# svg-project/Sparse-VideoGen

Hardware: AMD Instinct MI355X
Metric: attn_tflops_svg1_block_sparse (higher is better)
Workload: dtype bf16; 1 GPU; HunyuanVideo T2V hy720p SVG1 sparse layer-call: sample_mse(64 rows) + band attention with fused head placement, cfg=1 H=24 D=128 F=33 P=3600 ctx=256 prompt=64 S=119056 band=15616 density=0.2456; parallelism=single, variant=0, heads=alt

## Files before the change

include/svg_attn.h:

```cpp
#ifndef SVG_ATTN_H_
#define SVG_ATTN_H_

#include <stddef.h>
#include <stdint.h>

#ifdef __cplusplus
extern "C" {
#endif

#define SVG_DTYPE_BF16 0
#define SVG_DTYPE_F16 1
#define SVG_DTYPE_F32 2

#define SVG_OK 0
#define SVG_ERR_BAD_ARG (-1)
#define SVG_ERR_UNSUPPORTED (-2)
#define SVG_ERR_WORKSPACE (-3)
#define SVG_ERR_LAUNCH (-4)

#define SVG_ABI_VERSION 4
int svg_abi_version(void);

const char* svg_strerror(int code);
int svg_last_hip_error(void);
// ... 212 lines not shown
int svg_sample_mse_flagged(const void* q, const void* k, const void* v, const int64_t* rows, int32_t R, int32_t BH, int32_t S,
                           int32_t D, int32_t dtype, float sm_scale, const svg_profile_desc_t* prof, float* out_mse,
                           void* workspace, size_t workspace_bytes, const int32_t* skip_flag, void* stream);

size_t svg_band_attention_fp8_workspace_bytes(int32_t BH, int32_t S, int32_t D);
int svg_band_attention_fp8(const void* q, const void* k, const void* v, void* o, int32_t BH, int32_t S, int32_t D, int32_t dtype,
                           float sm_scale, const svg_band_mask_t* mask, const svg_perm_desc_t* perm, void* workspace,
                           size_t workspace_bytes, void* stream);
int svg_band_attention_fp8_stage(const void* q, const void* k, const void* v, void* o, int32_t BH, int32_t S, int32_t D, int32_t dtype,
                                 float sm_scale, const svg_band_mask_t* mask, const svg_perm_desc_t* perm, void* workspace,
                                 size_t workspace_bytes, int32_t stage, void* stream);

size_t svg_varblock_attention_fp8_workspace_bytes(int32_t Hq, int32_t Hkv, int32_t QB, int32_t KB, int32_t Sq, int32_t Skv, int32_t D);
int svg_varblock_attention_fp8(const void* q, const void* k, const void* v, void* o, int32_t Hq, int32_t Hkv, int32_t Sq, int32_t Skv,
                               int32_t D, int32_t dtype, float sm_scale, const uint8_t* block_map, const int32_t* q_sizes,
                               const int32_t* k_sizes, int32_t QB, int32_t KB, const int32_t* q_row_idx, const int32_t* kv_row_idx,
                               void* workspace, size_t workspace_bytes, void* stream);

int32_t svg_band_attention_notify_target(int32_t S, const svg_band_mask_t* mask);
int svg_band_attention_notify(const void* q, const void* k, const void* v, void* o, int32_t BH, int32_t S, int32_t D,
                              int32_t dtype, float sm_scale, const svg_band_mask_t* mask, const svg_perm_desc_t* perm,
                              int32_t* done_per_head, int32_t done_words, void* stream);
int svg_wait_counters(const int32_t* counters, int32_t n, int32_t target, void* stream);
int svg_wait_counters_deadline(const int32_t* counters, int32_t n, int32_t target, int32_t timeout_ms, int32_t* timed_out,
                               void* stream);
int32_t svg_band_attention_notify_layout(int32_t S, const svg_band_mask_t* mask, int32_t nseg, int32_t* row_bounds, int32_t* targets);
int svg_band_attention_notify_seg(const void* q, const void* k, const void* v, void* o, int32_t BH, int32_t S, int32_t D,
                                  int32_t dtype, float sm_scale, const svg_band_mask_t* mask, const svg_perm_desc_t* perm,
                                  int32_t* done, int32_t done_words, int32_t nseg, void* stream);
int svg_band_attention_prescaled_notify_seg(const void* q_scaled, const void* k, const void* v, void* o, int32_t BH, int32_t S,
                                            int32_t D, int32_t dtype, const svg_band_mask_t* mask, const svg_perm_desc_t* perm,
                                            int32_t* done, int32_t done_words, int32_t nseg, void* stream);

int svg_debug_pp_trace(uint64_t* out104);

int svg_debug_clock_probe(const int32_t* stop_flag, uint64_t* out2, int32_t max_ms, void* stream);

int svg_debug_wg_trace(uint64_t* out, int32_t n_workgroups);

#ifdef __cplusplus
}
#endif
#endif
```

sparse-videogen_amd/csrc/attention.hip:

```cpp
#include <algorithm>

#include "attn_core.h"
#include "attn_f8.h"
#include "attn_m16.h"
#include "band_policy.h"

namespace svg {

template <typename T, int D, int NW>
__global__ __launch_bounds__(NW * 64, 2) void band_attn_kernel(typename BandPolicy<T, D, NW>::Params prm) {
    extern __shared__ __attribute__((aligned(16))) char smem[];
    attn_body<T, D, NW, BandPolicy<T, D, NW>>(prm, smem, nullptr);
}

template <typename T, int D>
__global__ __launch_bounds__(512, (D == 64 ? 4 : 2)) void band_attn_pp2_kernel(typename BandPolicy<T, D, 8>::Params prm) {
    extern __shared__ __attribute__((aligned(16))) char smem[];
    attn_body_pp2<T, D, BandPolicy<T, D, 8>, false, 0, false, D == 64>(prm, smem, nullptr);
}
template <typename T>
__global__ __launch_bounds__(512, 4) void band_attn_pp2_switch64_kernel(typename BandPolicy<T, 64, 8>::Params prm,
                                                                        typename BandPolicy<T, 64, 8>::Params prm_alt,
                                                                        const int32_t* __restrict__ flag) {
    extern __shared__ __attribute__((aligned(16))) char smem[];
    if (flag[0] != 0) attn_body_pp2<T, 64, BandPolicy<T, 64, 8>, false, 0, false, true>(prm_alt, smem, nullptr);
    else attn_body_pp2<T, 64, BandPolicy<T, 64, 8>, false, 0, false, true>(prm, smem, nullptr);
}
template <typename T, int D>
__global__ __launch_bounds__(512, 2) void band_attn_pp2q_switch_kernel(typename BandPolicy<T, D, 8>::Params prm,
                                                                       typename BandPolicy<T, D, 8>::Params prm_alt,
                                                                       const int32_t* __restrict__ flag) {
    extern __shared__ __attribute__((aligned(16))) char smem[];
    if (flag[0] != 0) attn_body_pp2<T, D, BandPolicy<T, D, 8>, false, 0, true>(prm_alt, smem, nullptr);
    else attn_body_pp2<T, D, BandPolicy<T, D, 8>, false, 0, true>(prm, smem, nullptr);
}

__global__ __launch_bounds__(512, 2) void band_attn_pp2_frozen_kernel(typename BandPolicy<__bf16, 128, 8>::Params prm) {
    extern __shared__ __attribute__((aligned(16))) char smem[];
    attn_body_pp2<__bf16, 128, BandPolicy<__bf16, 128, 8>, false, 8>(prm, smem, nullptr);
}
template <typename T>
__global__ __launch_bounds__(512, 2) void band_attn_m16_kernel(typename BandPolicy<T, 128, 8>::Params prm) {
    extern __shared__ __attribute__((aligned(16))) char smem[];
    attn_body_m16<T, BandPolicy<T, 128, 8>, false, 1>(prm, smem, nullptr);
}
template <typename T>
__global__ __launch_bounds__(512, 2) void band_attn_m16q_kernel(typename BandPolicy<T, 128, 8>::Params prm) {
    extern __shared__ __attribute__((aligned(16))) char smem[];
    attn_body_m16<T, BandPolicy<T, 128, 8>, false, 1, true>(prm, smem, nullptr);
}
template <typename T, bool PRE = false>
__global__ __launch_bounds__(512, 2) void band_attn_m16_switch_kernel(typename BandPolicy<T, 128, 8>::Params prm,
                                                                      typename BandPolicy<T, 128, 8>::Params prm_alt,
                                                                      const int32_t* __restrict__ flag) {
    extern __shared__ __attribute__((aligned(16))) char smem[];
    if (flag[0] != 0) attn_body_m16<T, BandPolicy<T, 128, 8>, false, 1, PRE>(prm_alt, smem, nullptr);
    else attn_body_m16<T, BandPolicy<T, 128, 8>, false, 1, PRE>(prm, smem, nullptr);
}
template <typename T, int D>
__global__ __launch_bounds__(512, 2) void band_attn_pp2q_kernel(typename BandPolicy<T, D, 8>::Params prm) {
    extern __shared__ __attribute__((aligned(16))) char smem[];
    attn_body_pp2<T, D, BandPolicy<T, D, 8>, false, 0, true>(prm, smem, nullptr);
}
#ifdef SVG_ABLATIONS
template <typename T, int D, int ABL>
__global__ __launch_bounds__(512, 2) void band_attn_pp2_trace_kernel(typename BandPolicy<T, D, 8>::Params prm) {
    extern __shared__ __attribute__((aligned(16))) char smem[];
    attn_body_pp2<T, D, BandPolicy<T, D, 8>, true, ABL>(prm, smem, nullptr);
}
template <typename T>
__global__ __launch_bounds__(512, 2) void band_attn_m16_trace_kernel(typename BandPolicy<T, 128, 8>::Params prm) {
    extern __shared__ __attribute__((aligned(16))) char smem[];
    attn_body_m16<T, BandPolicy<T, 128, 8>, true>(prm, smem, nullptr);
}
template <typename T, int D>
__global__ __launch_bounds__(512, 2) void band_attn_pp2q_trace_kernel(typename BandPolicy<T, D, 8>::Params prm) {
    extern __shared__ __attribute__((aligned(16))) char smem[];
    attn_body_pp2<T, D, BandPolicy<T, D, 8>, true, 0, true>(prm, smem, nullptr);
}
#endif

constexpr int kVbMaxKB = 4032;
constexpr int kVbFull = 256;
// ... 593 lines not shown
static inline int band_default(int D) { return D == 128 ? kBandM16 : kBandPingPong; }

int band_waves_per_tile(int variant) {
    const int v = variant == kBandAuto ? kBandPingPong : variant;
    return v == kBandW4 ? 4 : ((v == kBandPingPong || v == kBandM16) ? 8 : -1);
}

}

using namespace svg;

__global__ __launch_bounds__(64) void wait_counters_kernel(const int32_t* __restrict__ counters, int n, int target) {
    for (int i = threadIdx.x; i < n; i += 64) {
        while (__hip_atomic_load(counters + i, __ATOMIC_ACQUIRE, __HIP_MEMORY_SCOPE_AGENT) < target) __builtin_amdgcn_s_sleep(32);
    }
}

__global__ __launch_bounds__(64) void wait_counters_deadline_kernel(const int32_t* __restrict__ counters, int n, int target,
                                                                    long long ticks, int32_t* __restrict__ timed_out) {
    const long long t0 = wall_clock64();
    for (int i = threadIdx.x; i < n; i += 64) {
        while (__hip_atomic_load(counters + i, __ATOMIC_ACQUIRE, __HIP_MEMORY_SCOPE_AGENT) < target) {
            if (wall_clock64() - t0 > ticks) {
                __hip_atomic_store(timed_out, 1, __ATOMIC_RELAXED, __HIP_MEMORY_SCOPE_SYSTEM);
                return;
            }
            __builtin_amdgcn_s_sleep(32);
        }
    }
}

static bool g_trace_is_w4 = false;

static int band_check_args(const void* q, const void* k, const void* v, const void* o, int32_t BH, int32_t S, int32_t D,
                           const svg_band_mask_t* mask, const svg_perm_desc_t* perm) {
    if (!q || !k || !v || !o || !mask || BH <= 0 || S <= 0) return SVG_ERR_BAD_ARG;
    if (const int rc = check_band_mask(S, mask, perm); rc != SVG_OK) return rc;
    if ((int64_t)BH * S * D >= (1ll << 40)) return SVG_ERR_UNSUPPORTED;
    return check_rows(S, D);
}

static int band_dispatch(const void* q, const void* k, const void* v, void* o, int32_t BH, int32_t S, int32_t D, int32_t dtype,
                         float sm_scale, const svg_band_mask_t* mask, const svg_perm_desc_t* perm, int32_t variant, BandOpts opts,
                         int32_t done_words, const svg_attn_layout_t* layout, void* stream) {
    int rc = band_check_args(q, k, v, o, BH, S, D, mask, perm);
    if (rc == SVG_OK && opts.alt_mask) rc = check_band_mask(S, opts.alt_mask, nullptr);
    if (rc != SVG_OK) return rc;
    if (opts.done && (int64_t)done_words < (int64_t)BH * (opts.done_nseg + 1)) return SVG_ERR_WORKSPACE;
    if (opts.strided && (rc = layout_from_abi(layout, BH, BH, S, S, D, q, k, v, o, opts.lay)) != SVG_OK) return rc;
    const hipStream_t st = (hipStream_t)stream;
    int trace_abl = -1;
    if ((variant & 0xFF) == 32) {
        opts.trace = true;
        opts.trace_abl = (variant >> 8) & 15;
        g_trace_is_w4 = true;
        return run_band_w4(q, k, v, o, BH, S, D, dtype, sm_scale, mask, perm, opts, st);
    }
    if (variant & 64) {
        trace_abl = (variant >> 8) & 15;
        variant = kBandPingPong;
        g_trace_is_w4 = false;
    }
    if (variant == kBandAuto) variant = band_default(D);
    if (opts.done && band_waves_per_tile(variant) < 0) return SVG_ERR_UNSUPPORTED;
    if (opts.strided && variant != kBandM16 && variant != kBandPingPong) return SVG_ERR_UNSUPPORTED;
    if (variant == kBandW4) return run_band_w4(q, k, v, o, BH, S, D, dtype, sm_scale, mask, perm, opts, st);
    if (variant != kBandLockstep4 && variant != kBandPingPong && variant != kBandFrozen && variant != kBandM16) return SVG_ERR_BAD_ARG;
    return dispatch_td(dtype, D, [&](auto t, auto d) -> int {
        using T = decltype(t);
        constexpr int DD = decltype(d)::value;
        using Pol = BandPolicy<T, DD, 8>;
        auto launch = [&](auto kern, int lds) {
            const typename Pol::Params p = make_band_params<Pol, T>(q, k, v, o, BH, S, sm_scale, mask, perm, opts);
            return launch_attn(kern, p, dim3(p.nqt * BH), 512, lds, st);
        };
        auto launch_switch = [&](auto kern, int lds) {
            const typename Pol::Params a = make_band_params<Pol, T>(q, k, v, o, BH, S, sm_scale, mask, perm, opts);
            const typename Pol::Params b = make_band_params<Pol, T>(q, k, v, o, BH, S, sm_scale, opts.alt_mask, nullptr, opts);
            if (const int r2 = configure_lds((const void*)kern, lds); r2 != SVG_OK) return r2;
            hipLaunchKernelGGL(kern, dim3(std::max(a.nqt, b.nqt) * BH), dim3(512), lds, st, a, b, opts.use_alt);
            return launch_status();
        };
        switch (variant) {
            case kBandLockstep4: {
                using Pol4 = BandPolicy<T, DD, 4>;
                const typename Pol4::Params p = make_band_params<Pol4, T>(q, k, v, o, BH, S, sm_scale, mask, perm, opts);
                return launch_attn(band_attn_kernel<T, DD, 4>, p, dim3(p.nqt * BH), 256, attn_lds_bytes<DD, 4>(), st);
            }
            case kBandPingPong:
#ifdef SVG_ABLATIONS
                if constexpr (DD == 128 && std::is_same<T, __bf16>::value) {
                    switch (trace_abl) {
#define SVG_PP_TRACE(A) case A: return launch(band_attn_pp2_trace_kernel<T, DD, A>, attn_pp2_lds_bytes<DD>());
                        SVG_PP_TRACE(0) SVG_PP_TRACE(1) SVG_PP_TRACE(2) SVG_PP_TRACE(4) SVG_PP_TRACE(5) SVG_PP_TRACE(6) SVG_PP_TRACE(7) SVG_PP_TRACE(8)
#undef SVG_PP_TRACE
                        case -1: break;
                        case 3: return launch(band_attn_pp2q_trace_kernel<T, DD>, attn_pp2_lds_bytes<DD>());
                        case 9: return launch(band_attn_m16_trace_kernel<T>, attn_m16_lds_bytes());
                        default: return SVG_ERR_UNSUPPORTED;
                    }
                }
#endif
                if (trace_abl >= 0) return SVG_ERR_UNSUPPORTED;
                if (opts.use_alt) {
                    if (opts.prescaled) return launch_switch(band_attn_pp2q_switch_kernel<T, DD>, attn_pp2_lds_bytes<DD>());
                    if constexpr (DD == 64) return launch_switch(band_attn_pp2_switch64_kernel<T>, attn_pp2_lds_bytes<64>());
                    return SVG_ERR_UNSUPPORTED;
                }
                return launch(opts.prescaled ? band_attn_pp2q_kernel<T, DD> : band_attn_pp2_kernel<T, DD>, attn_pp2_lds_bytes<DD>());
            case kBandFrozen:
                if constexpr (DD == 128 && std::is_same<T, __bf16>::value) {
                    if (opts.done || opts.prescaled) return SVG_ERR_UNSUPPORTED;
                    return launch(band_attn_pp2_frozen_kernel, attn_pp2_lds_bytes<128>());
                }
                return SVG_ERR_UNSUPPORTED;
            default:
                if constexpr (DD == 128) {
                    if (opts.use_alt)
                        return launch_switch(opts.prescaled ? band_attn_m16_switch_kernel<T, true> : band_attn_m16_switch_kernel<T>,
                                             attn_m16_lds_bytes());
                    return launch(opts.prescaled ? band_attn_m16q_kernel<T> : band_attn_m16_kernel<T>, attn_m16_lds_bytes());
                }
                return SVG_ERR_UNSUPPORTED;
        }
    });
}

extern "C" int svg_band_attention(const void* q, const void* k, const void* v, void* o, int32_t BH, int32_t S, int32_t D,
                                  int32_t dtype, float sm_scale, const svg_band_mask_t* mask,
                                  const svg_perm_desc_t* perm, int32_t variant, void* stream) {
    return band_dispatch(q, k, v, o, BH, S, D, dtype, sm_scale, mask, perm, variant, BandOpts(), 0, nullptr, stream);
}

extern "C" int svg_band_attention_strided(const void* q, const void* k, const void* v, void* o, int32_t BH, int32_t S, int32_t D,
                                          int32_t dtype, float sm_scale, const svg_band_mask_t* mask, const svg_perm_desc_t* perm,
                                          const svg_attn_layout_t* layout, void* stream) {
    BandOpts opts;
    opts.strided = true;
    return band_dispatch(q, k, v, o, BH, S, D, dtype, sm_scale, mask, perm, kBandAuto, opts, 0, layout, stream);
}

extern "C" int svg_band_attention_prescaled(const void* q_scaled, const void* k, const void* v, void* o, int32_t BH, int32_t S,
                                            int32_t D, int32_t dtype, const svg_band_mask_t* mask, const svg_perm_desc_t* perm,
                                            void* stream) {
    BandOpts opts;
    opts.prescaled = true;
    return band_dispatch(q_scaled, k, v, o, BH, S, D, dtype, 1.f, mask, perm, kBandAuto, opts, 0, nullptr, stream);
}

extern "C" int32_t svg_band_attention_notify_target(int32_t S, const svg_band_mask_t* mask) {
    if (!mask || S <= 0) return -1;
    using Pol = svg::BandPolicy<__bf16, 128, 8>;
    const auto p = svg::make_band_params<Pol, __bf16>(nullptr, nullptr, nullptr, nullptr, 1, S, 1.f, mask, nullptr);
    return p.nqt * band_waves_per_tile(kBandAuto);
// ... 63 lines not shown
}

static BandOpts switch_opts(const svg_band_mask_t* alt_mask, const int32_t* use_alt_flag) {
    BandOpts opts;
    opts.alt_mask = alt_mask, opts.use_alt = use_alt_flag;
    return opts;
}

extern "C" int svg_band_attention_switch(const void* q, const void* k, const void* v, void* o, int32_t BH, int32_t S, int32_t D,
                                         int32_t dtype, float sm_scale, const svg_band_mask_t* mask, const svg_perm_desc_t* perm,
                                         const svg_band_mask_t* alt_mask, const int32_t* use_alt_flag, void* stream) {
    if (!alt_mask || !use_alt_flag) return SVG_ERR_BAD_ARG;
    return band_dispatch(q, k, v, o, BH, S, D, dtype, sm_scale, mask, perm, kBandAuto, switch_opts(alt_mask, use_alt_flag), 0, nullptr,
                         stream);
}

extern "C" int svg_band_attention_switch_strided(const void* q, const void* k, const void* v, void* o, int32_t BH, int32_t S, int32_t D,
                                                 int32_t dtype, float sm_scale, const svg_band_mask_t* mask, const svg_perm_desc_t* perm,
                                                 const svg_band_mask_t* alt_mask, const int32_t* use_alt_flag,
                                                 const svg_attn_layout_t* layout, void* stream) {
    if (!layout || !alt_mask || !use_alt_flag) return SVG_ERR_BAD_ARG;
    BandOpts opts = switch_opts(alt_mask, use_alt_flag);
    opts.strided = true;
    return band_dispatch(q, k, v, o, BH, S, D, dtype, sm_scale, mask, perm, kBandAuto, opts, 0, layout, stream);
}

extern "C" int svg_band_attention_switch_prescaled(const void* q_scaled, const void* k, const void* v, void* o, int32_t BH, int32_t S,
                                                   int32_t D, int32_t dtype, const svg_band_mask_t* mask, const svg_perm_desc_t* perm,
                                                   const svg_band_mask_t* alt_mask, const int32_t* use_alt_flag, void* stream) {
    if (!alt_mask || !use_alt_flag) return SVG_ERR_BAD_ARG;
    BandOpts opts = switch_opts(alt_mask, use_alt_flag);
    opts.prescaled = true;
    return band_dispatch(q_scaled, k, v, o, BH, S, D, dtype, 1.f, mask, perm, kBandAuto, opts, 0, nullptr, stream);
}

extern "C" int svg_debug_wg_trace(uint64_t* out, int n_workgroups) {
#ifdef SVG_ABLATIONS
    if (!out || n_workgroups < 0 || n_workgroups > kWgTraceMax) return SVG_ERR_BAD_ARG;
    hipError_t e = hipMemcpyFromSymbol(out, HIP_SYMBOL(g_wg_trace), (size_t)n_workgroups * 6 * sizeof(uint64_t));
    if (e != hipSuccess) {
        g_last_hip_error = (int)e;
        return SVG_ERR_LAUNCH;
    }
    return SVG_OK;
#else
    (void)out, (void)n_workgroups;
    return SVG_ERR_UNSUPPORTED;
#endif
}

extern "C" int svg_debug_pp_trace(uint64_t* out104) {
#ifdef SVG_ABLATIONS
    if (!out104) return SVG_ERR_BAD_ARG;
    if (g_trace_is_w4) return w4_read_trace(out104);
    hipError_t e = hipMemcpyFromSymbol(out104, HIP_SYMBOL(g_pp_trace), 104 * sizeof(uint64_t));
    if (e != hipSuccess) {
        g_last_hip_error = (int)e;
        return SVG_ERR_LAUNCH;
    }
    return SVG_OK;
#else
    (void)out104;
    return SVG_ERR_UNSUPPORTED;
#endif
}

// ... 228 lines not shown
```

sparse-videogen_amd/csrc/attn_m16.h:

```cpp
#pragma once
#include "attn_core.h"

namespace svg {

template <typename T>
struct Mfma16;
template <>
struct Mfma16<__bf16> {
    static __device__ __forceinline__ f32x4 mfma(bf16x8 a, bf16x8 b, f32x4 c) { return __builtin_amdgcn_mfma_f32_16x16x32_bf16(a, b, c, 0, 0, 0); }
    static __device__ __forceinline__ f32x4 mfma_keep_c(bf16x8 a, bf16x8 b, const f32x4& c) {
        f32x4 d;
        asm volatile("v_mfma_f32_16x16x32_bf16 %0, %1, %2, %3" : "=&v"(d) : "v"(a), "v"(b), "v"(c));
        return d;
    }
};
template <>
struct Mfma16<_Float16> {
    static __device__ __forceinline__ f32x4 mfma(f16x8 a, f16x8 b, f32x4 c) { return __builtin_amdgcn_mfma_f32_16x16x32_f16(a, b, c, 0, 0, 0); }
    static __device__ __forceinline__ f32x4 mfma_keep_c(f16x8 a, f16x8 b, const f32x4& c) {
        f32x4 d;
        asm volatile("v_mfma_f32_16x16x32_f16 %0, %1, %2, %3" : "=&v"(d) : "v"(a), "v"(b), "v"(c));
        return d;
    }
};

constexpr int attn_m16_lds_bytes() { return attn_pp2_lds_bytes<128>(); }

__device__ __forceinline__ float quad_group_max(float x) {
    x = vmax2(x, __shfl_xor(x, 16));
    return vmax2(x, __shfl_xor(x, 32));
}
__device__ __forceinline__ float quad_group_sum(float x) {
    x += __shfl_xor(x, 16);
    return x + __shfl_xor(x, 32);
}

template <typename T, typename P, bool TRACE = false, int ONEBAR = -1, bool PRE = false>
__device__ __forceinline__ void attn_body_m16(const typename P::Params& prm, char* smem, char* policy_lds) {
    using E = Elt<T>;
    using M = Mfma16<T>;
    using V8 = typename E::v8;
    constexpr int D = 128;
    constexpr int NW = 8;
    constexpr int KS = D / 32;
    constexpr int NDB = D / 16;
    constexpr int NS = 4;
    constexpr int kImg = kBN * D * 2;
    constexpr int kStage = 2 * kImg;
    constexpr int NP = 2;
    constexpr int kCarry = 8;
    constexpr int kPF = 8;
    constexpr bool kOneBar = ONEBAR < 0 ? P::kOneBarrier : (ONEBAR != 0);
    static_assert(P::kRowBlocks == 1 && !P::kPartialOut && !P::kFixup && P::kIntervalMask, "band / variable-block policy");
    constexpr bool MSUM = std::is_same_v<T, __bf16> && !PRE;
    constexpr float kBias = MSUM ? 10.f : 0.f;

    typename P::Ctx ctx;
    if (!P::init(prm, ctx, policy_lds)) return;

    const int tid = threadIdx.x;
    const int lane = tid & 63;
    const int wave = wave_id();
    const int g4 = lane >> 4;
    const int n16 = lane & 15;
    const bool lagging = wave >= NW / 2;
    const int nT = ctx.nT;

    const T* __restrict__ qb = P::q_base(prm, ctx);
    const T* __restrict__ kb_ = P::k_base(prm, ctx);
    const T* __restrict__ vb = P::v_base(prm, ctx);
    const unsigned lds0 = (unsigned)(size_t)smem;

    const int dma_kg = wave / 2;
    const int dma_db0 = (wave % 2) * NP;
    const int krow = 16 * dma_kg + (lane >> 2);
    typename P::KvCursor cur;
    P::kv_cursor_init(prm, ctx, cur, krow);
    const unsigned vsw = (unsigned)((lane >> 4) & 1) << 1;
    const unsigned col_v = (unsigned)(dma_db0 * 64 + (((lane & 3) ^ vsw) * 16));
    const unsigned lds_piece = lds0 + (unsigned)(dma_db0 * (kBN * 64) + dma_kg * 1024);
    int nphys = 0, nnext = 0;
    auto resolve = [&](int t, auto guard_c) {
        if constexpr (decltype(guard_c)::value) nnext = (t < nT) ? P::kv_phys(prm, ctx, cur, t, krow) : 0;
        else nnext = P::kv_phys(prm, ctx, cur, t, krow);
    };
    constexpr std::true_type kGuarded{};
    auto take = [&]() { nphys = nnext; };
    const unsigned k_rsb = (unsigned)P::k_rs(prm) * 2u, v_rsb = (unsigned)P::v_rs(prm) * 2u;
    auto dma_piece = [&](int t, auto j_c) {
        constexpr int j = decltype(j_c)::value;
        const unsigned st = __builtin_amdgcn_readfirstlane(lds_piece + (unsigned)((t % NS) * kStage) + j * (kBN * 64));
        const unsigned ko = __umul24((unsigned)nphys, k_rsb) + col_v;
// ... 316 lines not shown
            }
#pragma unroll
        for (int b = 0; b < 4; ++b) asm volatile("" : "+v"(sc[b][0]), "+v"(sc[b][1]));
#pragma unroll
        for (int i = 0; i < kCarry; ++i) carry_load(0, i);
    }
    const int bar_n = lagging ? 1 : 0, bar_m = lagging ? 0 : 1;
    auto tile = [&](int t, auto has_next_c, auto guard_c) {
        tick(std::integral_constant<int, 0>{});
        if constexpr (kOneBar) pp_barrier_if(bar_n);
        else pp_barrier();
        tick(std::integral_constant<int, 1>{});
        vector_phase(t, guard_c);
        tick(std::integral_constant<int, 2>{});
        if constexpr (kOneBar) pp_barrier_if(bar_m);
        else pp_barrier();
        tick(std::integral_constant<int, 3>{});
        __builtin_amdgcn_s_setprio(1);
        matrix_phase(t, has_next_c);
        __builtin_amdgcn_s_setprio(0);
    };
    int t = 0;
    for (const int n_main = nT - dist - 1; t < n_main; ++t) tile(t, std::true_type{}, std::false_type{});
    for (; t + 1 < nT; ++t) tile(t, std::true_type{}, kGuarded);
    if (nT > 0) tile(nT - 1, std::false_type{}, kGuarded);
    pp_barrier();
    if (!kOneBar && !lagging) pp_barrier();
    if constexpr (TRACE) {
        if (blockIdx.x == kPpTraceBlock && lane == 0) {
#pragma unroll
            for (int j = 0; j < 4; ++j) g_pp_trace[wave * 8 + j] = tr_acc[j];
            if (wave == 0) g_pp_trace[64] = (unsigned long long)nT, g_pp_trace[65] = tr_last - tr_first;
        }
    }

    constexpr int kEpiStride = D * 2 + 8;
    char* erow = smem + (size_t)(wave * 32) * kEpiStride;
#pragma unroll
    for (int rb = 0; rb < 2; ++rb) {
        const float l_tot = MSUM ? acc_l[rb][0] : quad_group_sum(l_run[rb]);
        const float inv = l_tot > 0.f ? 1.f / l_tot : 0.f;
#pragma unroll
        for (int db = 0; db < NDB; ++db) {
            typename E::v4 o4;
#pragma unroll
            for (int j = 0; j < 4; ++j) o4[j] = E::from_float(acc_o[db][rb][j] * inv);
            *(typename E::v4*)(erow + (rb * 16 + n16) * kEpiStride + (16 * db + 4 * g4) * 2) = o4;
        }
    }
    __builtin_amdgcn_s_waitcnt(0xc07f);
    __builtin_amdgcn_wave_barrier();
    T* __restrict__ ob = P::o_base(prm, ctx);
    const int o_rs = P::o_rs(prm);
    constexpr int kLanesPerRow = D * 2 / 8;
    constexpr int kRowsPerPass = 64 / kLanesPerRow;
    const int sub = lane / kLanesPerRow;
    const int colb = (lane - sub * kLanesPerRow) * 8;
    int ephys[32 / kRowsPerPass];
#pragma unroll
    for (int i = 0; i < 32 / kRowsPerPass; ++i) ephys[i] = P::q_phys(prm, ctx, wave * 32 + i * kRowsPerPass + sub);
#pragma unroll
    for (int i = 0; i < 32 / kRowsPerPass; ++i) {
        const int rr = i * kRowsPerPass + sub;
        const u32x2 val = *(const u32x2*)(erow + rr * kEpiStride + colb);
        if (ephys[i] >= 0) *(u32x2*)((char*)(ob + (size_t)ephys[i] * o_rs) + colb) = val;
    }
    P::notify(prm, ctx);
}

}
```

sparse-videogen_amd/csrc/band_policy.h:

```cpp
#pragma once
#include <algorithm>

#include "attn_core.h"

namespace svg {

struct BandOpts {
    int32_t* done = nullptr;
    int done_nseg = 1;
    bool prescaled = false;
    bool trace = false;
    int trace_abl = 0;
    bool strided = false;
    AttnLayout lay{};
    const svg_band_mask_t* alt_mask = nullptr;
    const int32_t* use_alt = nullptr;
};

inline int check_band_mask(int S, const svg_band_mask_t* mask, const svg_perm_desc_t* perm) {
    if (mask->real_len < 0 || mask->real_len > S || mask->band < 0 || mask->band > S + 1) return SVG_ERR_BAD_ARG;
    if (mask->colfull_lo > mask->colfull_hi || mask->rowfull_lo > mask->rowfull_hi) return SVG_ERR_BAD_ARG;
    if (perm && perm->head_perm_flag) {
        if (perm->num_frame <= 0 || perm->frame_size <= 0 || perm->vid0 < 0 ||
            (int64_t)perm->vid0 + (int64_t)perm->num_frame * perm->frame_size > S)
// ... 47 lines not shown
    static __device__ __forceinline__ int phys_row(const Params& p, const Ctx& c, int logical) {
        if (c.perm) {
            const unsigned i = (unsigned)(logical - p.vid0);
            if (i < (unsigned)p.V) {
                const unsigned pp = i / (unsigned)p.F;
                const unsigned f = i - pp * (unsigned)p.F;
                return p.vid0 + (int)(f * (unsigned)p.P + pp);
            }
        }
        return logical;
    }

    static __device__ __forceinline__ bool init(const Params& p, Ctx& c, char*) {
        int qt;
        const int nh = p.BH * p.n_heavy;
        const int b = blockIdx.x;
        if (b >= p.nqt * p.BH) return false;
        if (b < nh) {
            c.head = b / p.n_heavy;
            qt = p.heavy_lo + (b - c.head * p.n_heavy);
        } else {
            const int b2 = b - nh;
            const int full = ((p.nqt * p.BH - nh) / (kNumXCD * 32)) * (kNumXCD * 32);
            int w2 = b2;
            if (b2 < full) {
                const int xcd = b2 % kNumXCD, s = b2 / kNumXCD;
                w2 = (s / 32) * (kNumXCD * 32) + xcd * 32 + (s % 32);
            }
            const int nl = p.nqt - p.n_heavy;
            c.head = w2 / nl;
            const int r = w2 - c.head * nl;
            qt = r < p.heavy_lo ? r : r + p.n_heavy;
        }
        const bool r1 = qt >= p.reg_t0[1], r2 = qt >= p.reg_t0[2], r3 = qt >= p.reg_t0[3];
        const int rlo = r3 ? p.reg_lo[3] : r2 ? p.reg_lo[2] : r1 ? p.reg_lo[1] : p.reg_lo[0];
        const int rhi = r3 ? p.reg_hi[3] : r2 ? p.reg_hi[2] : r1 ? p.reg_hi[1] : p.reg_hi[0];
        const int rt0 = r3 ? p.reg_t0[3] : r2 ? p.reg_t0[2] : r1 ? p.reg_t0[1] : 0;
        c.qt = qt;
        c.q0 = rlo + (qt - rt0) * BM;
        c.q_end = min(rhi, c.q0 + BM);
        c.perm = (p.head_flag != nullptr) && (p.head_flag[c.head] != 0);

        constexpr int BIG = 1 << 28;
        int alo = BIG, ahi = BIG, blo = BIG, bhi = BIG, clo = BIG, chi = BIG;
        const int real = p.real_len;
        if (c.q0 < real) {
            const int qr1 = min(c.q_end, real);
            if (c.q0 < p.rf_hi && qr1 > p.rf_lo) {
                alo = 0, ahi = (real + kBN - 1) / kBN;
            } else {
                alo = max(0, c.q0 - p.band + 1) / kBN;
                ahi = (min(real, qr1 - 1 + p.band) + kBN - 1) / kBN;
                const int ch = min(p.cf_hi, real);
                if (ch > p.cf_lo) blo = p.cf_lo / kBN, bhi = (ch + kBN - 1) / kBN;
            }
        }
        if (c.q_end > real) clo = real / kBN, chi = (p.S + kBN - 1) / kBN;
#define SVG_CSWAP(x, xh, y, yh) if (y < x) { int t_ = x; x = y; y = t_; t_ = xh; xh = yh; yh = t_; }
        SVG_CSWAP(alo, ahi, blo, bhi)
        SVG_CSWAP(blo, bhi, clo, chi)
        SVG_CSWAP(alo, ahi, blo, bhi)
#undef SVG_CSWAP
        if (blo < BIG && blo <= ahi) {
            ahi = max(ahi, bhi);
            blo = clo, bhi = chi, clo = BIG, chi = BIG;
            if (blo < BIG && blo <= ahi) ahi = max(ahi, bhi), blo = BIG, bhi = BIG;
        } else if (clo < BIG && clo <= bhi) {
            bhi = max(bhi, chi), clo = BIG, chi = BIG;
        }
        c.seg_lo[0] = alo, c.seg_n[0] = ahi - alo;
        c.seg_lo[1] = blo, c.seg_n[1] = bhi - blo;
        c.seg_lo[2] = clo, c.seg_n[2] = chi - clo;
        c.nT = c.seg_n[0] + c.seg_n[1] + c.seg_n[2];
        const int w0 = c.q0 + wave_id() * kWR, w1 = min(w0 + kWR, c.q_end);
        c.fk_lo = 1, c.fk_hi = 0;
        if (w0 < c.q_end && w1 <= real) {
            const bool full_rows = w0 >= p.rf_lo && w1 <= p.rf_hi;
            c.fk_lo = full_rows ? 0 : max(w1 - p.band, 0);
            c.fk_hi = min(full_rows ? real : w0 + p.band - kBN, min(real, p.S) - kBN);
        }
        return true;
    }

    static __device__ __forceinline__ const T* q_base(const Params& p, const Ctx& c) { return p.q + layout_head_off(p.lay.q_bs, p.lay.q_hs, p.lay.hpb_q, c.head); }
    static __device__ __forceinline__ const T* k_base(const Params& p, const Ctx& c) { return p.k + layout_head_off(p.lay.k_bs, p.lay.k_hs, p.lay.hpb_kv, c.head); }
    static __device__ __forceinline__ const T* v_base(const Params& p, const Ctx& c) { return p.v + layout_head_off(p.lay.v_bs, p.lay.v_hs, p.lay.hpb_kv, c.head); }
    static __device__ __forceinline__ T* o_base(const Params& p, const Ctx& c) { return p.o + layout_head_off(p.lay.o_bs, p.lay.o_hs, p.lay.hpb_q, c.head); }
    static __device__ __forceinline__ int q_rs(const Params& p) { return p.lay.q_rs; }
    static __device__ __forceinline__ int k_rs(const Params& p) { return p.lay.k_rs; }
    static __device__ __forceinline__ int v_rs(const Params& p) { return p.lay.v_rs; }
    static __device__ __forceinline__ int o_rs(const Params& p) { return p.lay.o_rs; }

    static __device__ __forceinline__ int q_logical(const Ctx& c, int row) { return c.q0 + row; }
    static __device__ __forceinline__ bool wave_active(const Ctx& c, int wrow0) { return c.q0 + wrow0 < c.q_end; }
    static __device__ __forceinline__ int q_phys(const Params& p, const Ctx& c, int row) {
        const int l = c.q0 + row;
        return l < c.q_end ? phys_row(p, c, l) : -1;
    }
    static __device__ __forceinline__ int tile_key0(const Ctx& c, int t) {
        const int n01 = c.seg_n[0] + c.seg_n[1];
        const int a = c.seg_lo[0] + t, b = c.seg_lo[1] + (t - c.seg_n[0]), d = c.seg_lo[2] + (t - n01);
        const int bd = t < n01 ? b : d;
        return (t < c.seg_n[0] ? a : bd) * kBN;
    }
    struct TileCur {
        int k0, left;
        int k1, left1;
        int k2, left2;
    };
    static __device__ __forceinline__ void tile_cur_shift(TileCur& tc) {
        tc.k0 = tc.k1, tc.left = tc.left1;
        tc.k1 = tc.k2, tc.left1 = tc.left2;
        tc.left2 = 0;
    }
// ... 116 lines not shown
                                                         unsigned& blen) {
        const int real = p.real_len;
        const bool rq = q < real;
        const bool rowf = (unsigned)(q - p.rf_lo) < (unsigned)(p.rf_hi - p.rf_lo);
        const int band_lo = max(q - p.band + 1, 0), band_hi = min(q + p.band, real);
        const int lo = rq ? (rowf ? 0 : band_lo) : real;
        const int hi = rq ? (rowf ? real : band_hi) : p.S;
        a0 = lo, alen = (unsigned)max(hi - lo, 0);
        const int ch = min(p.cf_hi, real);
        b0 = p.cf_lo, blen = (rq && !rowf) ? (unsigned)max(ch - p.cf_lo, 0) : 0u;
    }
    static __device__ __forceinline__ float score_fixup(const Params&, float s) { return s; }
    static __device__ __forceinline__ void notify(const Params& p, const Ctx& c) {
        if (p.done) {
            asm volatile("s_waitcnt vmcnt(0)" ::: "memory");
            __threadfence();
            if ((threadIdx.x & 63) == 0) {
                int32_t* cnt = p.done + c.head * p.done_nseg;
                if (!c.perm) {
                    atomicAdd(cnt + min(c.qt / p.done_tps, p.done_nseg - 1), 1);
                } else if (atomicAdd(p.done + p.BH * p.done_nseg + c.head, 1) == p.nqt * NW - 1) {
                    __threadfence();
                    for (int sgm = 0; sgm < p.done_nseg; ++sgm) {
                        const int t_lo = sgm * p.done_tps;
                        const int t_hi = (sgm == p.done_nseg - 1) ? p.nqt : min(p.nqt, (sgm + 1) * p.done_tps);
                        atomicAdd(cnt + sgm, (t_hi - t_lo) * NW);
                    }
                }
            }
        }
    }
};

inline int configure_lds(const void* kernel, int lds) {
    struct Entry {
        const void* kernel;
        int device, lds;
    };
    static thread_local Entry table[64];
    static thread_local int n = 0;
    int dev = 0;
    if (hipGetDevice(&dev) != hipSuccess) dev = 0;
    Entry* e = nullptr;
    for (int i = 0; i < n; ++i)
        if (table[i].kernel == kernel && table[i].device == dev) e = &table[i];
    if (e && e->lds >= lds) return SVG_OK;
    const hipError_t err = hipFuncSetAttribute(kernel, hipFuncAttributeMaxDynamicSharedMemorySize, lds);
    if (err != hipSuccess) {
        g_last_hip_error = (int)err;
        return SVG_ERR_LAUNCH;
    }
    if (e) e->lds = lds;
    else if (n < 64) table[n++] = Entry{kernel, dev, lds};
    return SVG_OK;
}

template <typename K, typename Prm>
inline int launch_attn(K kernel, const Prm& prm, dim3 grid, int threads, int lds, hipStream_t st) {
    const int rc = configure_lds((const void*)kernel, lds);
    if (rc != SVG_OK) return rc;
    hipLaunchKernelGGL(kernel, grid, dim3(threads), lds, st, prm);
    return launch_status();
}

template <typename Pol, typename T>
inline typename Pol::Params make_band_params(const void* q, const void* k, const void* v, void* o, int BH, int S, float sm_scale,
// ... 57 lines not shown
```

sparse-videogen_amd/svg/_native.py:

```python
from __future__ import annotations

import ctypes as C
import os
from pathlib import Path
from typing import NamedTuple, Optional, Sequence

import torch

_LIB_PATH = Path(__file__).resolve().parent.parent / "lib" / "libsvgattn.so"
_lib: Optional[C.CDLL] = None
_load_error: Optional[str] = None

SVG_DTYPE_BF16, SVG_DTYPE_F16 = 0, 1


class BandMask(C.Structure):

    _fields_ = [
        ("real_len", C.c_int32),
        ("band", C.c_int32),
        ("colfull_lo", C.c_int32),
        ("colfull_hi", C.c_int32),
        ("rowfull_lo", C.c_int32),
        ("rowfull_hi", C.c_int32),
# ... 31 lines not shown
    _fields_ = [
        ("vid0", C.c_int32),
        ("num_frame", C.c_int32),
        ("frame_size", C.c_int32),
        ("emulate_bf16", C.c_int32),
        ("variant", ProfileVariant * 2),
    ]


_I32, _I64, _F32, _VP, _SZ = C.c_int32, C.c_int64, C.c_float, C.c_void_p, C.c_size_t


class PrologueSegment(C.Structure):
    _fields_ = [("q_in", C.c_void_p), ("k_in", C.c_void_p), ("v_in", C.c_void_p), ("rows", C.c_int32), ("norm_kind", C.c_int32),
                ("q_weight", C.c_void_p), ("q_bias", C.c_void_p), ("k_weight", C.c_void_p), ("k_bias", C.c_void_p), ("eps", C.c_float)]


class TensorStrides(C.Structure):
    _fields_ = [("batch", C.c_int64), ("head", C.c_int64), ("row", C.c_int64)]


class AttnLayout(C.Structure):
    _fields_ = [("heads_per_batch", C.c_int32), ("kv_heads_per_batch", C.c_int32), ("q", TensorStrides), ("k", TensorStrides),
                ("v", TensorStrides), ("o", TensorStrides)]


SIGNATURES = {
    "svg_abi_version": (C.c_int, []),
    "svg_strerror": (C.c_char_p, [C.c_int]),
    "svg_last_hip_error": (C.c_int, []),
    "svg_build_info": (C.c_char_p, []),
    "svg_debug_pp_trace": (C.c_int, [_VP]),
    "svg_debug_wg_trace": (C.c_int, [_VP, _I32]),
    "svg_rms_norm_forward": (C.c_int, [_VP, _VP, C.c_int64, _I32, _I32, C.c_float, _VP]),
    "svg_layer_norm_forward": (C.c_int, [_VP, _VP, _VP, C.c_int64, _I32, _I32, _VP]),
    "svg_apply_qk_rope_inplace_cossin": (C.c_int, [_VP, _VP, _VP, _VP, _I32, _I32, _I32, _I32, _I32, _I32, _I32, _VP]),
    "svg_apply_qk_rope_inplace_cossin_txtlast": (C.c_int, [_VP, _VP, _VP, _VP, _I32, _I32, _I32, _I32, _I32, _I32, _I32, _VP]),
    "svg_apply_qk_rope_inplace_cossin_complex": (C.c_int, [_VP, _VP, _VP, _VP, _I32, _I32, _I32, _I32, _I32, _I32, _I32, _VP]),
    "svg_bsr_to_block_map": (C.c_int, [_VP, _VP, _I32, _I32, _I32, _I32, _I32, _I32, _VP, _VP, _VP, _VP]),
    "svg_layernorm_forward": (C.c_int, [_VP, _VP, _VP, _VP, C.c_int64, _I32, _I32, _I32, _I32, C.c_float, _VP]),
    "svg_rmsnorm_forward": (C.c_int, [_VP, _VP, _VP, C.c_int64, _I32, _I32, _I32, _I32, C.c_float, _VP]),
    "svg_layernorm_forward_ex": (C.c_int, [_VP, _VP, _VP, _VP, C.c_int64, _I32, _I32, _I32, _I32, C.c_float, _I32, _VP]),
    "svg_modulate_shift_forward": (C.c_int, [_VP, _VP, _VP, _VP, C.c_int64, _I32, C.c_int64, _I32, _I32, _VP]),
    "svg_modulate_gate_residual_forward": (C.c_int, [_VP, _VP, _VP, _VP, C.c_int64, _I32, C.c_int64, _I32, _I32, _I32, _VP]),
    "svg_layernorm_modulate_forward": (C.c_int, [_VP, _VP, _VP, _VP, _VP, _VP, C.c_int64, _I32, C.c_int64, _I32, _I32, _I32,
                                                 C.c_float, _VP]),
    "svg_layernorm_modulate_forward_ex": (C.c_int, [_VP, _VP, _VP, _VP, _VP, _VP, C.c_int64, _I32, C.c_int64, _I32, _I32, _I32,
                                                    C.c_float, _I32, _VP]),
    "svg_qk_norm_rope_transpose": (C.c_int, [_VP, _VP, _VP, _VP, _I32, _I32, _I32, _I32, _I32, _I32, _I32, _VP, _VP, _VP, _VP,
                                             C.c_float, _I32, _VP, _VP, _I32, _I32, _VP]),
    "svg_qk_norm_rope": (C.c_int, [_VP, _VP, _I32, _I32, _I32, _I32, _I32, _I32, _I32, _VP, _VP, _VP, _VP, C.c_float, _I32, _VP,
                                   _VP, _I32, _I32, _VP]),
    "svg_qk_norm_rope_qscale": (C.c_int, [_VP, _VP, _I32, _I32, _I32, _I32, _I32, _I32, _I32, _VP, _VP, _VP, _VP, C.c_float, _I32, _VP,
                                          _VP, _I32, _I32, C.c_float, _VP]),
    "svg_qk_norm_rope_transpose_qscale": (C.c_int, [_VP, _VP, _VP, _VP, _I32, _I32, _I32, _I32, _I32, _I32, _I32, _VP, _VP, _VP, _VP,
                                                    C.c_float, _I32, _VP, _VP, _I32, _I32, C.c_float, _VP]),
    "svg_qk_norm_rope_transpose_joint": (C.c_int, [C.POINTER(PrologueSegment), _I32, _VP, _VP, _VP, _I32, _I32, _I32, _I32, _I32, _VP, _VP,
                                                   _I32, _I32, C.c_float, _VP]),
    "svg_rmsnorm_rope_transpose": (C.c_int, [_VP, _VP, _VP, _VP, _VP, _VP, _I32, _I32, _I32, _I32, _I32, _VP, _VP, _I32, C.c_float, _I32, _VP,
                                             _VP, _I32, _I32, C.c_float, _VP]),
    "svg_head_placement": (C.c_int, [_VP, _VP, _I32, _VP, _I32, _I32, _I32, _I32, _I32, _I32, _I32, _I32, _I32, _VP]),
    "svg_permute_rows": (C.c_int, [_VP, _VP, _VP, _I32, _I32, _I32, _I32, _VP]),
    "svg_inverse_permute_rows": (C.c_int, [_VP, _VP, _VP, _I32, _I32, _I32, _I32, _VP]),
    "svg_argsort_workspace_bytes": (_SZ, [_I32, _I32, _I32]),
    "svg_argsort_labels": (C.c_int, [_VP, _VP, _VP, _I32, _I32, _I32, _VP, _SZ, _VP]),
    "svg_band_attention": (C.c_int, [_VP, _VP, _VP, _VP, _I32, _I32, _I32, _I32, _F32, C.POINTER(BandMask),
# ... 991 lines not shown
```

Measured before the change: 1269 TFLOP/s.

## Add persistent per-XCD atomic work queue for m16 band attention tiles

Replaces the one-workgroup-per-tile launch of the m16 band attention kernel with a persistent kernel sized to the CU count. Workgroups pull (head, q-tile) items from per-XCD atomic counters, starting with heavy tiles, then chunked light tiles, and finally a shared tail of the longest edge tiles. The aim is better load balance and XCD-local L2 reuse across uneven tile costs. In exchange it adds atomic and barrier overhead per tile, a per-stream device counter block that must reset itself at the end of each launch, and it falls back to the old launch during graph capture or when notify counters are in use.

```diff
diff --git a/include/svg_attn.h b/include/svg_attn.h
--- a/include/svg_attn.h
+++ b/include/svg_attn.h
@@ -268,6 +268,9 @@
                                             int32_t D, int32_t dtype, const svg_band_mask_t* mask, const svg_perm_desc_t* perm,
                                             int32_t* done, int32_t done_words, int32_t nseg, void* stream);
 
+int32_t svg_band_queue_order(int32_t BH, int32_t S, const svg_band_mask_t* mask, int32_t* out, int32_t out_words);
+int svg_debug_band_queue_cap(int32_t max_workgroups);
+
 int svg_debug_pp_trace(uint64_t* out104);
 
 int svg_debug_clock_probe(const int32_t* stop_flag, uint64_t* out2, int32_t max_ms, void* stream);
diff --git a/sparse-videogen_amd/csrc/attention.hip b/sparse-videogen_amd/csrc/attention.hip
--- a/sparse-videogen_amd/csrc/attention.hip
+++ b/sparse-videogen_amd/csrc/attention.hip
@@ -1,4 +1,6 @@
 #include <algorithm>
+#include <atomic>
+#include <mutex>
 
 #include "attn_core.h"
 #include "attn_f8.h"
@@ -49,6 +51,30 @@
     extern __shared__ __attribute__((aligned(16))) char smem[];
     attn_body_m16<T, BandPolicy<T, 128, 8>, false, 1, true>(prm, smem, nullptr);
 }
+template <typename T, bool PRE = false>
+__global__ __launch_bounds__(512, 2) void band_attn_m16_queue_kernel(typename BandPolicy<T, 128, 8>::Params prm, BandQueue qd) {
+    extern __shared__ __attribute__((aligned(16))) char smem[];
+    using Pol = BandPolicy<T, 128, 8>;
+    int* const slot = (int*)(smem + attn_m16_lds_bytes());
+    int dry = 0;
+    for (;;) {
+        if (threadIdx.x == 0) {
+            const int xcd = __builtin_amdgcn_s_getreg((31 << 11) | 20) & (kNumXCD - 1);
+            int head = -1, qt = 0;
+            const int w = qd.take(xcd, dry);
+            if (w >= 0) qd.decode(w, head, qt);
+            slot[0] = head, slot[1] = qt;
+        }
+        __syncthreads();
+        const int head = __builtin_amdgcn_readfirstlane(slot[0]), qt = __builtin_amdgcn_readfirstlane(slot[1]);
+        if (head < 0) break;
+        typename Pol::Ctx ctx;
+        Pol::init_tile(prm, ctx, head, qt);
+        attn_m16_tile<T, Pol, false, 1, PRE>(prm, ctx, smem);
+    }
+    if (threadIdx.x == 0) qd.leave(gridDim.x);
+}
+constexpr int kQueueLds = 16;
 template <typename T, bool PRE = false>
 __global__ __launch_bounds__(512, 2) void band_attn_m16_switch_kernel(typename BandPolicy<T, 128, 8>::Params prm,
                                                                       typename BandPolicy<T, 128, 8>::Params prm_alt,
@@ -708,6 +734,60 @@
 
 static bool g_trace_is_w4 = false;
 
+namespace {
+constexpr int kQueueBlocks = 64;
+constexpr int kQueueDevices = 16;
+struct QueuePool {
+    int device = -1, n_cu = 0, n_used = 0;
+    int32_t* base = nullptr;
+    hipStream_t owner[kQueueBlocks];
+};
+std::mutex g_queue_mu;
+QueuePool g_queue_pool[kQueueDevices];
+int g_queue_pools = 0;
+std::atomic<int> g_queue_cap{0};
+}
+
+int32_t* svg::band_queue_block(hipStream_t st, int& n_cu) {
+    hipStreamCaptureStatus cap = hipStreamCaptureStatusNone;
+    if (hipStreamIsCapturing(st, &cap) != hipSuccess || cap != hipStreamCaptureStatusNone) {
+        (void)hipGetLastError();
+        return nullptr;
+    }
+    int dev = 0;
+    if (hipGetDevice(&dev) != hipSuccess) return nullptr;
+    std::lock_guard<std::mutex> lock(g_queue_mu);
+    QueuePool* pool = nullptr;
+    for (int i = 0; i < g_queue_pools; ++i)
+        if (g_queue_pool[i].device == dev) pool = &g_queue_pool[i];
+    if (!pool) {
+        if (g_queue_pools == kQueueDevices) return nullptr;
+        int n = 0;
+        void* mem = nullptr;
+        const size_t bytes = (size_t)kQueueBlocks * kQueueWords * sizeof(int32_t);
+        if (hipDeviceGetAttribute(&n, hipDeviceAttributeMultiprocessorCount, dev) != hipSuccess || n <= 0 ||
+            hipMalloc(&mem, bytes) != hipSuccess) {
+            (void)hipGetLastError();
+            return nullptr;
+        }
+        if (hipMemset(mem, 0, bytes) != hipSuccess || hipDeviceSynchronize() != hipSuccess) {
+            (void)hipGetLastError();
+            (void)hipFree(mem);
+            return nullptr;
+        }
+        pool = &g_queue_pool[g_queue_pools++];
+        pool->device = dev, pool->n_cu = n, pool->base = (int32_t*)mem;
+    }
+    n_cu = pool->n_cu;
+    for (int i = 0; i < pool->n_used; ++i)
+        if (pool->owner[i] == st) return pool->base + (size_t)i * kQueueWords;
+    if (pool->n_used == kQueueBlocks) return nullptr;
+    pool->owner[pool->n_used] = st;
+    return pool->base + (size_t)(pool->n_used++) * kQueueWords;
+}
+
+int svg::band_queue_cap() { return g_queue_cap.load(std::memory_order_relaxed); }
+
 static int band_check_args(const void* q, const void* k, const void* v, const void* o, int32_t BH, int32_t S, int32_t D,
                            const svg_band_mask_t* mask, const svg_perm_desc_t* perm) {
     if (!q || !k || !v || !o || !mask || BH <= 0 || S <= 0) return SVG_ERR_BAD_ARG;
@@ -749,6 +829,20 @@
         auto launch = [&](auto kern, int lds) {
             const typename Pol::Params p = make_band_params<Pol, T>(q, k, v, o, BH, S, sm_scale, mask, perm, opts);
             return launch_attn(kern, p, dim3(p.nqt * BH), 512, lds, st);
+        };
+        auto launch_queue = [&](auto kern_q, auto kern, int lds) {
+            const typename Pol::Params p = make_band_params<Pol, T>(q, k, v, o, BH, S, sm_scale, mask, perm, opts);
+            int n_cu = 0;
+            int32_t* const block = opts.done ? nullptr : band_queue_block(st, n_cu);
+            const int cap = band_queue_cap();
+            if (!block || (p.nqt * BH <= n_cu && cap == 0)) return launch_attn(kern, p, dim3(p.nqt * BH), 512, lds, st);
+            BandQueue qd = make_band_queue<Pol>(p);
+            qd.ctr = block;
+            int n_wg = std::min(qd.n_items, n_cu);
+            if (cap > 0) n_wg = std::min(n_wg, cap);
+            if (const int r2 = configure_lds((const void*)kern_q, lds + kQueueLds); r2 != SVG_OK) return r2;
+            hipLaunchKernelGGL(kern_q, dim3(n_wg), dim3(512), lds + kQueueLds, st, p, qd);
+            return launch_status();
         };
         auto launch_switch = [&](auto kern, int lds) {
             const typename Pol::Params a = make_band_params<Pol, T>(q, k, v, o, BH, S, sm_scale, mask, perm, opts);
@@ -795,7 +889,8 @@
                     if (opts.use_alt)
                         return launch_switch(opts.prescaled ? band_attn_m16_switch_kernel<T, true> : band_attn_m16_switch_kernel<T>,
                                              attn_m16_lds_bytes());
-                    return launch(opts.prescaled ? band_attn_m16q_kernel<T> : band_attn_m16_kernel<T>, attn_m16_lds_bytes());
+                    if (opts.prescaled) return launch_queue(band_attn_m16_queue_kernel<T, true>, band_attn_m16q_kernel<T>, attn_m16_lds_bytes());
+                    return launch_queue(band_attn_m16_queue_kernel<T>, band_attn_m16_kernel<T>, attn_m16_lds_bytes());
                 }
                 return SVG_ERR_UNSUPPORTED;
         }
@@ -925,6 +1020,34 @@
     BandOpts opts = switch_opts(alt_mask, use_alt_flag);
     opts.prescaled = true;
     return band_dispatch(q_scaled, k, v, o, BH, S, D, dtype, 1.f, mask, perm, kBandAuto, opts, 0, nullptr, stream);
+}
+
+extern "C" int32_t svg_band_queue_order(int32_t BH, int32_t S, const svg_band_mask_t* mask, int32_t* out, int32_t out_words) {
+    if (!mask || BH <= 0 || S <= 0 || check_band_mask(S, mask, nullptr) != SVG_OK) return -1;
+    using Pol = svg::BandPolicy<__bf16, 128, 8>;
+    const auto p = svg::make_band_params<Pol, __bf16>(nullptr, nullptr, nullptr, nullptr, BH, S, 1.f, mask, nullptr);
+    const BandQueue qd = svg::make_band_queue<Pol>(p);
+    if (!out) return qd.n_items;
+    int n = 0;
+    for (int x = 0; x <= kNumXCD; ++x)
+        for (unsigned i = 0;; ++i) {
+            const int w = x < kNumXCD ? qd.item(x, i) : qd.tail_item(i);
+            if (w < 0) break;
+            if (3 * (n + 1) > out_words) return -1;
+            int head, qt;
+            qd.decode(w, head, qt);
+            Pol::Ctx c;
+            Pol::kv_schedule(p, c, qt);
+            out[3 * n] = x, out[3 * n + 1] = head * p.nqt + qt, out[3 * n + 2] = c.nT;
+            ++n;
+        }
+    return n;
+}
+
+extern "C" int svg_debug_band_queue_cap(int32_t max_workgroups) {
+    if (max_workgroups < 0) return SVG_ERR_BAD_ARG;
+    g_queue_cap.store(max_workgroups, std::memory_order_relaxed);
+    return SVG_OK;
 }
 
 extern "C" int svg_debug_wg_trace(uint64_t* out, int n_workgroups) {
diff --git a/sparse-videogen_amd/csrc/attn_m16.h b/sparse-videogen_amd/csrc/attn_m16.h
--- a/sparse-videogen_amd/csrc/attn_m16.h
+++ b/sparse-videogen_amd/csrc/attn_m16.h
@@ -36,7 +36,7 @@
 }
 
 template <typename T, typename P, bool TRACE = false, int ONEBAR = -1, bool PRE = false>
-__device__ __forceinline__ void attn_body_m16(const typename P::Params& prm, char* smem, char* policy_lds) {
+__device__ __forceinline__ void attn_m16_tile(const typename P::Params& prm, const typename P::Ctx& ctx, char* smem) {
     using E = Elt<T>;
     using M = Mfma16<T>;
     using V8 = typename E::v8;
@@ -55,9 +55,8 @@
     constexpr bool MSUM = std::is_same_v<T, __bf16> && !PRE;
     constexpr float kBias = MSUM ? 10.f : 0.f;
 
-    typename P::Ctx ctx;
-    if (!P::init(prm, ctx, policy_lds)) return;
-
+    unsigned long long wg_t0 = 0, wg_t2 = 0;
+    if constexpr (TRACE) wg_t0 = __builtin_amdgcn_s_memtime();
     const int tid = threadIdx.x;
     const int lane = tid & 63;
     const int wave = wave_id();
@@ -440,6 +439,7 @@
             for (int j = 0; j < 4; ++j) g_pp_trace[wave * 8 + j] = tr_acc[j];
             if (wave == 0) g_pp_trace[64] = (unsigned long long)nT, g_pp_trace[65] = tr_last - tr_first;
         }
+        wg_t2 = __builtin_amdgcn_s_memtime();
     }
 
     constexpr int kEpiStride = D * 2 + 8;
@@ -474,6 +474,22 @@
         if (ephys[i] >= 0) *(u32x2*)((char*)(ob + (size_t)ephys[i] * o_rs) + colb) = val;
     }
     P::notify(prm, ctx);
+    if constexpr (TRACE) {
+        asm volatile("s_waitcnt vmcnt(0)" ::: "memory");
+        if (wave == 0 && lane == 0 && blockIdx.x < (unsigned)kWgTraceMax) {
+            unsigned long long* w = g_wg_trace + (size_t)blockIdx.x * 6;
+            w[0] = wg_t0, w[1] = tr_first, w[2] = wg_t2, w[3] = __builtin_amdgcn_s_memtime();
+            w[4] = __builtin_amdgcn_s_getreg((31 << 11) | 4);
+            w[5] = __builtin_amdgcn_s_getreg((31 << 11) | 20);
+        }
+    }
 }
 
+template <typename T, typename P, bool TRACE = false, int ONEBAR = -1, bool PRE = false>
+__device__ __forceinline__ void attn_body_m16(const typename P::Params& prm, char* smem, char* policy_lds) {
+    typename P::Ctx ctx;
+    if (!P::init(prm, ctx, policy_lds)) return;
+    attn_m16_tile<T, P, TRACE, ONEBAR, PRE>(prm, ctx, smem);
 }
+
+}
diff --git a/sparse-videogen_amd/csrc/band_policy.h b/sparse-videogen_amd/csrc/band_policy.h
--- a/sparse-videogen_amd/csrc/band_policy.h
+++ b/sparse-videogen_amd/csrc/band_policy.h
@@ -103,6 +103,27 @@
             const int r = w2 - c.head * nl;
             qt = r < p.heavy_lo ? r : r + p.n_heavy;
         }
+        init_tile(p, c, c.head, qt);
+        return true;
+    }
+
+    static __device__ __forceinline__ void init_tile(const Params& p, Ctx& c, int head, int qt) {
+        c.head = head;
+        c.perm = (p.head_flag != nullptr) && (p.head_flag[c.head] != 0);
+        kv_schedule(p, c, qt);
+        const int real = p.real_len;
+        const int w0 = c.q0 + wave_id() * kWR, w1 = min(w0 + kWR, c.q_end);
+        c.fk_lo = 1, c.fk_hi = 0;
+        if (w0 < c.q_end && w1 <= real) {
+            const bool full_rows = w0 >= p.rf_lo && w1 <= p.rf_hi;
+            c.fk_lo = full_rows ? 0 : max(w1 - p.band, 0);
+            c.fk_hi = min(full_rows ? real : w0 + p.band - kBN, min(real, p.S) - kBN);
+        }
+    }
+
+    static __host__ __device__ __forceinline__ void kv_schedule(const Params& p, Ctx& c, int qt) {
+        using std::max;
+        using std::min;
         const bool r1 = qt >= p.reg_t0[1], r2 = qt >= p.reg_t0[2], r3 = qt >= p.reg_t0[3];
         const int rlo = r3 ? p.reg_lo[3] : r2 ? p.reg_lo[2] : r1 ? p.reg_lo[1] : p.reg_lo[0];
         const int rhi = r3 ? p.reg_hi[3] : r2 ? p.reg_hi[2] : r1 ? p.reg_hi[1] : p.reg_hi[0];
@@ -110,7 +131,6 @@
         c.qt = qt;
         c.q0 = rlo + (qt - rt0) * BM;
         c.q_end = min(rhi, c.q0 + BM);
-        c.perm = (p.head_flag != nullptr) && (p.head_flag[c.head] != 0);
 
         constexpr int BIG = 1 << 28;
         int alo = BIG, ahi = BIG, blo = BIG, bhi = BIG, clo = BIG, chi = BIG;
@@ -143,14 +163,6 @@
         c.seg_lo[1] = blo, c.seg_n[1] = bhi - blo;
         c.seg_lo[2] = clo, c.seg_n[2] = chi - clo;
         c.nT = c.seg_n[0] + c.seg_n[1] + c.seg_n[2];
-        const int w0 = c.q0 + wave_id() * kWR, w1 = min(w0 + kWR, c.q_end);
-        c.fk_lo = 1, c.fk_hi = 0;
-        if (w0 < c.q_end && w1 <= real) {
-            const bool full_rows = w0 >= p.rf_lo && w1 <= p.rf_hi;
-            c.fk_lo = full_rows ? 0 : max(w1 - p.band, 0);
-            c.fk_hi = min(full_rows ? real : w0 + p.band - kBN, min(real, p.S) - kBN);
-        }
-        return true;
     }
 
     static __device__ __forceinline__ const T* q_base(const Params& p, const Ctx& c) { return p.q + layout_head_off(p.lay.q_bs, p.lay.q_hs, p.lay.hpb_q, c.head); }
@@ -333,6 +345,118 @@
     }
 };
 
+constexpr int kQueueChunk = 32;
+constexpr int kQueueTail = 256;
+constexpr int kQueueStride = 16;
+constexpr int kQueueCounters = kNumXCD + 2;
+constexpr int kQueueWords = kQueueCounters * kQueueStride;
+
+struct BandQueue {
+    int32_t* ctr;
+    int n_items;
+    int BH, nh, n_heavy, heavy_lo;
+    int nl;
+    int e_lo, e_hi;
+    int r0;
+    int n_tail;
+
+    __host__ __device__ int edge_tile(int rank, bool back) const { return back ? nl - e_hi + rank : e_lo - 1 - rank; }
+    __host__ __device__ void decode(int w, int& head, int& qt) const {
+        if (w < nh) {
+            head = w / n_heavy;
+            qt = heavy_lo + (w - head * n_heavy);
+            return;
+        }
+        int w2 = w - nh, r = 0;
+        const int nf = nl - e_lo - e_hi;
+        head = 0;
+        if (w >= n_items - n_tail) {
+            w2 = w - (n_items - n_tail);
+            const int m = e_lo < e_hi ? e_lo : e_hi;
+            const int both = m > r0 ? (m - r0) * 2 * BH : 0;
+            if (w2 < both) {
+                const int rank = r0 + w2 / (2 * BH), j = w2 % (2 * BH);
+                head = j >> 1;
+                r = edge_tile(rank, j & 1);
+            } else {
+                w2 -= both;
+                head = w2 % BH;
+                r = edge_tile((m > r0 ? m : r0) + w2 / BH, e_hi > e_lo);
+            }
+        } else if (w2 < BH * nf) {
+            head = w2 / nf;
+            r = e_lo + (w2 - head * nf);
+        } else {
+            w2 -= BH * nf;
+            const int b_lo = e_lo < r0 ? e_lo : r0, b_hi = e_hi < r0 ? e_hi : r0;
+            for (int t0 = 0; t0 < r0; t0 += kQueueChunk) {
+                const int cl = b_lo - t0 < 0 ? 0 : (b_lo - t0 > kQueueChunk ? kQueueChunk : b_lo - t0);
+                const int ct = b_hi - t0 < 0 ? 0 : (b_hi - t0 > kQueueChunk ? kQueueChunk : b_hi - t0);
+                const int c = cl + ct;
+                if (w2 < BH * c) {
+                    head = w2 / c;
+                    const int j = w2 - head * c;
+                    r = j < cl ? edge_tile(t0 + j, false) : edge_tile(t0 + j - cl, true);
+                    break;
+                }
+                w2 -= BH * c;
+            }
+        }
+        qt = r < heavy_lo ? r : r + n_heavy;
+    }
+    __host__ __device__ int item(int xcd, unsigned i) const {
+        if (i >= (unsigned)n_items) return -1;
+        const int nhx = nh > xcd ? (nh - xcd + kNumXCD - 1) / kNumXCD : 0;
+        if ((int)i < nhx) return xcd + kNumXCD * (int)i;
+        const int i2 = (int)i - nhx;
+        const int w = nh + ((i2 / kQueueChunk) * kNumXCD + xcd) * kQueueChunk + i2 % kQueueChunk;
+        return w < n_items - n_tail ? w : -1;
+    }
+    __host__ __device__ int tail_item(unsigned i) const { return i < (unsigned)n_tail ? n_items - n_tail + (int)i : -1; }
+    __device__ int take(int xcd, int& k) const {
+        for (; k < kNumXCD; ++k) {
+            const int x = (xcd + k) & (kNumXCD - 1);
+            const int w = item(x, (unsigned)atomicAdd(ctr + x * kQueueStride, 1));
+            if (w >= 0) return w;
+        }
+        if (k == kNumXCD) {
+            const int w = tail_item((unsigned)atomicAdd(ctr + kNumXCD * kQueueStride, 1));
+            if (w >= 0) return w;
+            ++k;
+        }
+        return -1;
+    }
+    __device__ void leave(int n_wg) const {
+        __threadfence();
+        if (atomicAdd(ctr + (kQueueCounters - 1) * kQueueStride, 1) == n_wg - 1) {
+            for (int x = 0; x < kQueueCounters; ++x) atomicExch(ctr + x * kQueueStride, 0);
+        }
+    }
+};
+
+template <typename Pol>
+inline BandQueue make_band_queue(const typename Pol::Params& p) {
+    BandQueue qd{};
+    qd.n_items = p.BH * p.nqt, qd.BH = p.BH;
+    qd.n_heavy = p.n_heavy, qd.heavy_lo = p.heavy_lo, qd.nh = p.BH * p.n_heavy, qd.nl = p.nqt - p.n_heavy;
+    int longest = -1, first = 0, last = -1;
+    for (int r = 0; r < qd.nl; ++r) {
+        typename Pol::Ctx c;
+        Pol::kv_schedule(p, c, r < p.heavy_lo ? r : r + p.n_heavy);
+        if (c.nT > longest) longest = c.nT, first = r;
+        if (c.nT == longest) last = r;
+    }
+    qd.e_lo = first, qd.e_hi = qd.nl - 1 - last;
+    if (qd.nl == 0) qd.e_lo = qd.e_hi = 0;
+    const int ranks = std::max(qd.e_lo, qd.e_hi);
+    qd.r0 = std::max(0, ranks - (kQueueTail + 2 * p.BH - 1) / (2 * p.BH));
+    qd.n_tail = p.BH * (std::max(0, qd.e_lo - qd.r0) + std::max(0, qd.e_hi - qd.r0));
+    return qd;
+}
+
+int32_t* band_queue_block(hipStream_t st, int& n_cu);
+int band_queue_cap();
+
 inline int configure_lds(const void* kernel, int lds) {
     struct Entry {
         const void* kernel;
diff --git a/sparse-videogen_amd/svg/_native.py b/sparse-videogen_amd/svg/_native.py
--- a/sparse-videogen_amd/svg/_native.py
+++ b/sparse-videogen_amd/svg/_native.py
@@ -87,6 +87,8 @@
     "svg_build_info": (C.c_char_p, []),
     "svg_debug_pp_trace": (C.c_int, [_VP]),
     "svg_debug_wg_trace": (C.c_int, [_VP, _I32]),
+    "svg_band_queue_order": (_I32, [_I32, _I32, C.POINTER(BandMask), _VP, _I32]),
+    "svg_debug_band_queue_cap": (C.c_int, [_I32]),
     "svg_rms_norm_forward": (C.c_int, [_VP, _VP, C.c_int64, _I32, _I32, C.c_float, _VP]),
     "svg_layer_norm_forward": (C.c_int, [_VP, _VP, _VP, C.c_int64, _I32, _I32, _VP]),
     "svg_apply_qk_rope_inplace_cossin": (C.c_int, [_VP, _VP, _VP, _VP, _I32, _I32, _I32, _I32, _I32, _I32, _I32, _VP]),
```

Measured after the change: 1298 TFLOP/s, median of 6. 2.3% higher.
